# videosegmentation/video_segment

Measured on AMD Instinct MI355X. Metric: over-segmented frames/sec at 1080p, higher is better.
Workload: dtype f32

## Files before the change

video_segment_amd/csrc/merge_stage.hip:

```cpp
#include <sched.h>
#include <time.h>

#include <algorithm>
#include <atomic>
#include <chrono>
#include <thread>
#include <vector>

#include "merge_common.h"
#include "scan_device.h"

namespace vsg {

__global__ __launch_bounds__(256) void k_build_bucket_table(const ListDesc* __restrict__ lists,
                                                             int num_lists,
                                                             int32_t* __restrict__ bucket_base) {
  const int b = blockIdx.x * 256 + threadIdx.x;
  if (b > kNumBuckets) return;
  int acc = 0;
  int32_t* row = bucket_base + (size_t)b * (num_lists + 1);
  for (int l = 0; l < num_lists; ++l) {
    row[l] = acc;
    const int32_t* off = lists[l].offsets;
    if (off) acc += off[b + 1] - off[b];
  }
  row[num_lists] = acc;
}

void LaunchBuildBucketTable(const ListDesc* lists, int num_lists, int32_t* bucket_base,
                            hipStream_t s) {
  hipLaunchKernelGGL(k_build_bucket_table, dim3((kNumBuckets + 1 + 255) / 256), dim3(256), 0, s,
                     lists, num_lists, bucket_base);
  VSG_HIP(hipGetLastError());
}

__global__ __launch_bounds__(256) void k_init_identity(int32_t* a, size_t n) {
  const size_t i = (size_t)blockIdx.x * 256 + threadIdx.x;
  if (i < n) a[i] = (int32_t)i;
}

void LaunchInitIdentity(int32_t* a, size_t n, hipStream_t s) {
  hipLaunchKernelGGL(k_init_identity, dim3((unsigned)((n + 255) / 256)), dim3(256), 0, s, a, n);
  VSG_HIP(hipGetLastError());
}

__global__ void k_mail_post(unsigned long long* slot, unsigned seq, const int32_t* p0, const int32_t* p1,
                            const int32_t* p2, const int32_t* p3) {
  if (p0) MailPost(slot, seq, 0, *p0);
  if (p1) MailPost(slot, seq, 1, *p1);
  if (p2) MailPost(slot, seq, 2, *p2);
  if (p3) MailPost(slot, seq, 3, *p3);
}

void LaunchMailPost(const MailSlot& slot, const int32_t* p0, const int32_t* p1, const int32_t* p2,
                    const int32_t* p3, hipStream_t s) {
  hipLaunchKernelGGL(k_mail_post, dim3(1), dim3(1), 0, s, slot.dev, slot.seq, p0, p1, p2, p3);
  VSG_HIP(hipGetLastError());
}

static std::atomic<int> g_live_graphs{0};
void MailRegisterGraph(int delta) { g_live_graphs.fetch_add(delta, std::memory_order_relaxed); }

static int UsableCores() {
  cpu_set_t set;
  CPU_ZERO(&set);
  if (sched_getaffinity(0, sizeof(set), &set) == 0 && CPU_COUNT(&set) > 0) return (int)CPU_COUNT(&set);
  const unsigned h = std::thread::hardware_concurrency();
  return h ? (int)h : 1;
}

int MailYieldMode() {
  if (const char* e = getenv("VSG_MAIL_YIELD")) return std::max(0, std::min(2, atoi(e)));
  return 2 * g_live_graphs.load(std::memory_order_relaxed) > UsableCores() ? 1 : 0;
}

static thread_local MailWaitCounters t_mail_counters;
MailWaitCounters MailWaitSnapshot() { return t_mail_counters; }
void MailWaitResetLongest() { t_mail_counters.longest_ms = 0; }

namespace {
struct MailWaitTimer {
  std::chrono::steady_clock::time_point t0 = std::chrono::steady_clock::now();
  ~MailWaitTimer() {
    const double ms = std::chrono::duration<double, std::milli>(std::chrono::steady_clock::now() - t0).count();
    t_mail_counters.waits += 1;
    t_mail_counters.wait_ms += ms;
    if (ms > t_mail_counters.longest_ms) t_mail_counters.longest_ms = ms;
  }
};
}

void MailWait(const MailSlot& slot, int count, int* values, hipStream_t s) {
  using clk = std::chrono::steady_clock;
  MailWaitTimer wait_timer;
  clk::time_point t0;
  bool timed = false;
  const int mode = MailYieldMode();
  constexpr unsigned long long kBriefSpins = 512;
  long sleep_ns = 20000;
  for (int i = 0; i < count; ++i) {
    for (unsigned long long spins = 0;; ++spins) {
      const unsigned long long w = slot.host[i];
      if ((unsigned)(w >> 32) == slot.seq) {
        values[i] = (int)(unsigned)(w & 0xffffffffull);
        break;
      }
#if defined(__x86_64__)
      __builtin_ia32_pause();
#endif
      if (mode != 0 && spins >= kBriefSpins) {
        if (mode == 1) {
          std::this_thread::yield();
        } else {
          const timespec ts = {0, sleep_ns};
          nanosleep(&ts, nullptr);
          sleep_ns = std::min(sleep_ns * 2, 200000l);
        }
      }
      if ((mode == 0 && (spins & 0xffffull) == 0xffffull) || (mode != 0 && (spins & 0x3ffull) == 0x3ffull)) {
        const hipError_t e = hipStreamQuery(s);
        if (e != hipSuccess && e != hipErrorNotReady) VSG_HIP(e);
        if (!timed) {
          t0 = clk::now();
          timed = true;
        } else if (e == hipSuccess && clk::now() - t0 > std::chrono::seconds(2)) {
          const unsigned long long w2 = slot.host[i];
          if ((unsigned)(w2 >> 32) != slot.seq) throw Error(-4 , "mailbox: a value never arrived");
        }
        if (mode == 0) std::this_thread::yield();
      }
    }
  }
}

static void DrainStreams(MergeScratch& S) {
  VSG_HIP(hipStreamSynchronize(S.main_stream));
  if (S.aux_stream) VSG_HIP(hipStreamSynchronize(S.aux_stream));
  if (S.aux2_stream) VSG_HIP(hipStreamSynchronize(S.aux2_stream));
}

int32_t* TakeZeroed(MergeScratch& S, size_t n) {
  ZeroPool& z = *S.zeros;
  n = (n + 3) & ~(size_t)3;
  VSG_REQUIRE(z.cap > 2 * kZeroArenaInts, -4, "zero pool: too small");
  const size_t half = (z.cap - kZeroArenaInts) / 2;
  VSG_REQUIRE(n <= half, -4, "zero pool: request too large");
  if (z.used + n > half) {
    DrainStreams(S);
    z.second_half = !z.second_half;
    z.used = 0;
    VSG_HIP(hipMemsetAsync(z.base + kZeroArenaInts + (z.second_half ? half : 0), 0, half * sizeof(int32_t),
                           S.main_stream));
  }
  int32_t* p = z.base + kZeroArenaInts + (z.second_half ? half : 0) + z.used;
  z.used += n;
  return p;
}

int32_t* TakeStageScalars(MergeScratch& S, size_t n) {
  ZeroPool& z = *S.zeros;
  n = (n + 3) & ~(size_t)3;
  VSG_REQUIRE(n <= kZeroArenaInts, -4, "zero pool: stage scalars too large");
  if (z.arena_used + n > kZeroArenaInts) {
    DrainStreams(S);
    VSG_HIP(hipMemsetAsync(z.base, 0, kZeroArenaInts * sizeof(int32_t), S.main_stream));
    z.arena_used = 0;
  }
  int32_t* p = z.base + z.arena_used;
  z.arena_used += n;
  return p;
}

constexpr int kFilterPer = 2;
constexpr int kFilterEdges = 256 * kFilterPer;

__global__ __launch_bounds__(256) void k_filter(int bucket, int bucket_hi, int j0, int n_b,
                                                 const ListDesc* __restrict__ lists,
                                                 const int32_t* __restrict__ bucket_base,
                                                 const int32_t* __restrict__ bucket_prefix,
                                                 const uint32_t* __restrict__ list_slot_base,
                                                 uint8_t* __restrict__ kept_all, NodeArrays nodes,
                                                 MergeParams P, int inert_mode,
                                                 int32_t* __restrict__ cc,
                                                 int32_t* __restrict__ e_ra,
                                                 int32_t* __restrict__ e_rb,
                                                 uint32_t* __restrict__ e_gpos,
                                                 FilterMasks M,
                                                 int32_t* __restrict__ num_ti, FilterSegs segs, int hubs,
                                                 int32_t* __restrict__ num_hub, int32_t* __restrict__ hub_excl,
                                                 float split_s) {
  __shared__ int wave_cnt[kFilterPer][4], wave_kept[kFilterPer][4];
  __shared__ int s_start[kFilterEdges], s_pos0[kFilterEdges];
  __shared__ const uint32_t* s_slots[kFilterEdges];
  __shared__ const int32_t* s_prev[kFilterEdges];
  __shared__ int s_type[kFilterEdges], s_base_a[kFilterEdges], s_base_b[kFilterEdges];
  __shared__ uint32_t s_slot_base[kFilterEdges];
  const int jf = blockIdx.x * kFilterEdges;
  int m_segs = 0;
  if (segs.start) {
    int first = 0;
    if (segs.n > kFilterEdges) {
      const int stride = (segs.n + 255) / 256;
      const int t1 = threadIdx.x * stride;
      const int c1 = __syncthreads_count(t1 < segs.n && segs.start[t1] <= jf);
      const int base = (c1 - 1) * stride;
      const int t2 = base + threadIdx.x;
      const int c2 = __syncthreads_count(threadIdx.x < stride && t2 < segs.n && segs.start[t2] <= jf);
      first = base + c2 - 1;
    }
    m_segs = min(kFilterEdges, segs.n - first);
    for (int i = threadIdx.x; i < m_segs; i += 256) {
      s_start[i] = segs.start[first + i];
      const int l = segs.list[first + i];
      s_pos0[i] = segs.pos0[first + i];
      const ListDesc L = lists[l];
      s_slots[i] = L.slots;
      s_prev[i] = L.type != 0 ? L.prev_idx : reinterpret_cast<const int32_t*>(L.slots);
      s_type[i] = L.type;
      s_base_a[i] = L.base_a;
      s_base_b[i] = L.base_b;
      s_slot_base[i] = list_slot_base[l];
    }
    __syncthreads();
  }
  bool valid[kFilterPer];
  int a[kFilterPer], b[kFilterPer], l_type[kFilterPer];
  uint32_t gpos[kFilterPer];
  if (segs.start) {
    const uint32_t* slots_p[kFilterPer];
    const int32_t* prev_p[kFilterPer];
    int pos[kFilterPer], base_a[kFilterPer], base_b[kFilterPer];
#pragma unroll
    for (int e = 0; e < kFilterPer; ++e) {
      const int j = jf + e * 256 + threadIdx.x;
      valid[e] = j < n_b;
      const int jc = valid[e] ? j : n_b - 1;
      int lo = 0, hi = m_segs;
      while (hi - lo > 1) {
        const int mid = (lo + hi) >> 1;
        if (s_start[mid] <= jc) lo = mid; else hi = mid;
      }
      pos[e] = s_pos0[lo] + (jc - s_start[lo]);
      slots_p[e] = s_slots[lo];
      prev_p[e] = s_prev[lo];
      l_type[e] = s_type[lo];
      base_a[e] = s_base_a[lo];
      base_b[e] = s_base_b[lo];
      gpos[e] = s_slot_base[lo] + (uint32_t)pos[e];
    }
    uint32_t slot[kFilterPer];
#pragma unroll
    for (int e = 0; e < kFilterPer; ++e) slot[e] = slots_p[e][pos[e]];
    uint32_t pix[kFilterPer];
    int pv[kFilterPer];
#pragma unroll
    for (int e = 0; e < kFilterPer; ++e) {
      const uint32_t tm = (uint32_t)-(int)(l_type[e] != 0);
      pix[e] = ((slot[e] / 9u) & tm) | ((slot[e] >> 2) & ~tm);
      pv[e] = prev_p[e][pix[e]];
    }
#pragma unroll
    for (int e = 0; e < kFilterPer; ++e) {
      a[e] = base_a[e] + (int)pix[e];
      const int kt = (int)(slot[e] - pix[e] * 9u);
      const int dy = kt / 3 - 1, dx = kt - (kt / 3) * 3 - 1;
      const int bt = base_b[e] + pv[e] + dy * P.W + dx;
      const int ks = (int)(slot[e] & 3u);
      const int bs = a[e] + (ks != 0 ? P.W : 0) + (ks == 0 || ks == 3 ? 1 : 0) - (ks == 2 ? 1 : 0);
      const int tm = -(int)(l_type[e] != 0);
      b[e] = (bt & tm) | (bs & ~tm);
    }
  } else {
#pragma unroll
    for (int e = 0; e < kFilterPer; ++e) {
      const int j = jf + e * 256 + threadIdx.x;
      valid[e] = j < n_b;
      const int jc = valid[e] ? j : n_b - 1;
      int bk = bucket;
      int jb = j0 + jc;
      if (bucket_hi > bucket + 1) {
        const int jg = bucket_prefix[bucket] + jb;
        int lo = bucket, hi = bucket_hi;
        while (hi - lo > 1) {
          const int mid = (lo + hi) >> 1;
          if (bucket_prefix[mid] <= jg) lo = mid; else hi = mid;
        }
        bk = lo;
        jb = jg - bucket_prefix[bk];
      }
      const int32_t* base_row = bucket_base + (size_t)bk * (P.num_lists + 1);
      const int l = LocateList(base_row, P.num_lists, jb);
      const int pos = lists[l].offsets[bk] + (jb - base_row[l]);
      const ListDesc L = lists[l];
      l_type[e] = L.type;
      DecodeEdge(L, L.slots[pos], P.W, a[e], b[e]);
      gpos[e] = list_slot_base[l] + (uint32_t)pos;
    }
  }
  constexpr int kChains = 2 * kFilterPer;
  int x0[kChains], root[kChains];
#pragma unroll
  for (int e = 0; e < kFilterPer; ++e) {
    x0[2 * e] = a[e];
    x0[2 * e + 1] = b[e];
  }
#pragma unroll
  for (int c = 0; c < kChains; ++c) root[c] = x0[c];
  for (bool any = true; any;) {
    int p[kChains];
#pragma unroll
    for (int c = 0; c < kChains; ++c) p[c] = nodes.parent[root[c]];
    any = false;
#pragma unroll
    for (int c = 0; c < kChains; ++c) {
      if (p[c] != root[c]) {
        root[c] = p[c];
        any = true;
      }
    }
  }
  {
    int cur[kChains];
#pragma unroll
    for (int c = 0; c < kChains; ++c) cur[c] = x0[c];
    for (bool any = true; any;) {
      int nx[kChains];
#pragma unroll
      for (int c = 0; c < kChains; ++c) nx[c] = cur[c] != root[c] ? nodes.parent[cur[c]] : root[c];
      any = false;
#pragma unroll
      for (int c = 0; c < kChains; ++c) {
        if (cur[c] != root[c]) {
          if (nx[c] != root[c]) nodes.parent[cur[c]] = root[c];
          cur[c] = nx[c];
          any = any || (cur[c] != root[c]);
        }
      }
    }
  }
  int ti[kFilterPer], active[kFilterPer], settled[kFilterPer];
#pragma unroll
  for (int e = 0; e < kFilterPer; ++e) {
    ti[e] = active[e] = settled[e] = 0;
    const int ra = root[2 * e], rb = root[2 * e + 1];
    if (!valid[e] || ra == rb) continue;
    if (P.spatial_survivors && l_type[e] == 0 && !P.spatial_survivors[gpos[e]]) continue;
    bool inert = false;
    int f1 = 0, f2 = 0, s1 = 0, s2 = 0, c1 = -1, c2 = -1;
    if (inert_mode != 0) {
      f1 = nodes.flags[ra];
      f2 = nodes.flags[rb];
      if (f1 & kFlagFinalized) s1 = __float_as_int(nodes.desc_sz[ra].w);
      if (f2 & kFlagFinalized) s2 = __float_as_int(nodes.desc_sz[rb].w);
      const bool both_final_large = (f1 & kFlagFinalized) && (f2 & kFlagFinalized) &&
                                    (s1 >= P.min_region_size) && (s2 >= P.min_region_size);
      if (inert_mode == 1) {
        inert = both_final_large;
      } else {
        c1 = nodes.cons[ra];
        c2 = nodes.cons[rb];
        if (c1 >= 0 && c2 >= 0) {
          inert = (c1 != c2);
        } else {
          inert = both_final_large;
        }
        if (inert) {
          ti[e] = 1;
          if (!(f1 & kFlagTentative)) nodes.flags[ra] = (uint8_t)(f1 | kFlagTentative);
          if (!(f2 & kFlagTentative)) nodes.flags[rb] = (uint8_t)(f2 | kFlagTentative);
        }
      }
    }
    if (inert) {
      kept_all[gpos[e]] = 1;
      settled[e] = 1;
    } else {
      active[e] = 1;
      bool hub_edge = false;
      if (hubs) {
        constexpr int kNoHub = kFlagNoDesc | kFlagHubExcluded;
        const bool h1 = (f1 & kFlagFinalized) && !(f1 & kNoHub) && s1 >= P.min_region_size;
        const bool h2 = (f2 & kFlagFinalized) && !(f2 & kNoHub) && s2 >= P.min_region_size;
        if (h1 != h2) {
          const int h = h1 ? ra : rb, x = h1 ? rb : ra;
          const int fx = h1 ? f2 : f1, cx = h1 ? c2 : c1, fh = h1 ? f1 : f2;
          const int ch = h1 ? c1 : c2;
          if ((cx < 0 || cx == ch) && !(fx & kFlagNoDesc)) {
            hub_edge = true;
            root[2 * e] = x;
            root[2 * e + 1] = h;
            if (!nodes.hub8[h]) nodes.hub8[h] = 1;
            if (!(*num_hub & 1)) atomicOr(num_hub, 1);
            if (cx >= 0) {
              const float4 dx = nodes.desc_sz[x], dh = nodes.desc_sz[h];
              const float u = dh.x - dx.x, v = dh.y - dx.y, w = dh.z - dx.z;
              if ((u * u + v * v + w * w) * (1.0f / 3.0f) > split_s) {
                HubViolationAt(hub_excl, 0, jf + e * 256 + (int)threadIdx.x);
                if (!(*num_hub & 16)) atomicOr(num_hub, 16);
              }
            }
          } else {
            HubViolationAt(hub_excl, 0, jf + e * 256 + (int)threadIdx.x);
            if (!(fh & kFlagHubBroken)) HubExclude(hub_excl, nodes.flags, h);
          }
        } else if (h1 && h2) {
          HubViolationAt(hub_excl, 0, jf + e * 256 + (int)threadIdx.x);
          if (s1 <= s2 && !(f1 & kFlagHubBroken)) HubExclude(hub_excl, nodes.flags, ra);
          if (s2 <= s1 && !(f2 & kFlagHubBroken)) HubExclude(hub_excl, nodes.flags, rb);
        }
      }
      if (!hub_edge) CcUnion(cc, ra, rb);
    }
  }
  const int w = threadIdx.x >> 6, lane = threadIdx.x & 63;
  const int n_blocks = (n_b + 255) >> 8;
  unsigned long long ma[kFilterPer], ms[kFilterPer];
#pragma unroll
  for (int e = 0; e < kFilterPer; ++e) {
    ma[e] = __ballot(active[e] != 0);
    ms[e] = __ballot(settled[e] != 0);
    const unsigned long long mt = __ballot(ti[e] != 0);
    const int vb = blockIdx.x * kFilterPer + e;
    if (lane == 0 && vb < n_blocks) {
      const size_t gw = (size_t)vb * 4 + w;
      M.active[gw] = ma[e];
      M.settled[gw] = ms[e];
      M.tentative[gw] = mt;
      wave_cnt[e][w] = (int)__popcll(ma[e]);
      wave_kept[e][w] = (int)__popcll(ma[e] | ms[e]);
      if (mt != 0 && *num_ti == 0) *num_ti = 1;
    }
  }
  __syncthreads();
#pragma unroll
  for (int e = 0; e < kFilterPer; ++e) {
    const int vb = blockIdx.x * kFilterPer + e;
    if (active[e] | settled[e]) {
      int rank = (int)__popcll((ma[e] | ms[e]) & ((1ull << lane) - 1ull));
      for (int k = 0; k < w; ++k) rank += wave_kept[e][k];
      const int slot = vb * 256 + rank;
      e_ra[slot] = root[2 * e];
      e_rb[slot] = root[2 * e + 1];
      e_gpos[slot] = gpos[e];
    }
    if (threadIdx.x == 0 && vb < n_blocks) {
      M.block_cnt[vb] = wave_cnt[e][0] + wave_cnt[e][1] + wave_cnt[e][2] + wave_cnt[e][3];
    }
  }
}

__device__ __forceinline__ int FilterSlot(const FilterMasks& M, int j) {
  const int block = j >> 8, w = (j >> 6) & 3, lane = j & 63;
  const size_t gw0 = (size_t)block * 4;
  int rank = (int)__popcll((M.active[gw0 + w] | M.settled[gw0 + w]) & ((1ull << lane) - 1ull));
  for (int k = 0; k < w; ++k) rank += (int)__popcll(M.active[gw0 + k] | M.settled[gw0 + k]);
  return block * 256 + rank;
}

__global__ __launch_bounds__(256) void k_clear_tentative(int n_b, FilterMasks M,
                                                          const int32_t* __restrict__ e_ra,
                                                          const int32_t* __restrict__ e_rb,
                                                          NodeArrays nodes) {
  const int j = blockIdx.x * 256 + threadIdx.x;
  if (j >= n_b || !((M.tentative[j >> 6] >> (j & 63)) & 1ull)) return;
  const int slot = FilterSlot(M, j);
  int r[2] = {e_ra[slot], e_rb[slot]};
  for (int k = 0; k < 2; ++k) {
    int x = r[k];
    for (;;) {
      const int f = nodes.flags[x];
      if (f & kFlagTentative) nodes.flags[x] = (uint8_t)(f & ~kFlagTentative);
      const int p = nodes.parent[x];
      if (p == x) break;
      x = p;
    }
  }
}

__global__ __launch_bounds__(256) void k_backup_roots(int n, const int32_t* __restrict__ a_ra,
                                                       const int32_t* __restrict__ a_rb,
                                                       NodeArrays nodes, float4* __restrict__ bk_ds,
                                                       int32_t* __restrict__ bk_cons,
                                                       uint8_t* __restrict__ bk_flags,
                                                       unsigned long long* __restrict__ stats) {
  const int i = blockIdx.x * 256 + threadIdx.x;
  if (i < 8) stats[8 + i] = stats[i];
  if (i >= n) return;
  const int ra = a_ra[i], rb = a_rb[i];
  bk_ds[2 * i] = nodes.desc_sz[ra];
  bk_cons[2 * i] = nodes.cons[ra];
  bk_flags[2 * i] = nodes.flags[ra];
  bk_ds[2 * i + 1] = nodes.desc_sz[rb];
  bk_cons[2 * i + 1] = nodes.cons[rb];
  bk_flags[2 * i + 1] = nodes.flags[rb];
}

__global__ __launch_bounds__(256) void k_restore_roots(int n, const int32_t* __restrict__ a_ra,
                                                        const int32_t* __restrict__ a_rb,
                                                        NodeArrays nodes,
                                                        const float4* __restrict__ bk_ds,
                                                        const int32_t* __restrict__ bk_cons,
                                                        const uint8_t* __restrict__ bk_flags,
                                                        unsigned long long* __restrict__ stats) {
  const int i = blockIdx.x * 256 + threadIdx.x;
  if (i < 8) stats[i] = stats[8 + i];
  if (i >= n) return;
  const int ra = a_ra[i], rb = a_rb[i];
  nodes.parent[ra] = ra;
  nodes.desc_sz[ra] = bk_ds[2 * i];
  nodes.cons[ra] = bk_cons[2 * i];
  nodes.flags[ra] = bk_flags[2 * i];
  nodes.parent[rb] = rb;
  nodes.desc_sz[rb] = bk_ds[2 * i + 1];
  nodes.cons[rb] = bk_cons[2 * i + 1];
  nodes.flags[rb] = bk_flags[2 * i + 1];
}

__global__ __launch_bounds__(256) void k_clear_kept(int n_b, FilterMasks M,
                                                     const uint32_t* __restrict__ e_gpos,
                                                     uint8_t* __restrict__ kept_all) {
  const int j = blockIdx.x * 256 + threadIdx.x;
  if (j >= n_b) return;
  if (((M.active[j >> 6] | M.settled[j >> 6]) >> (j & 63)) & 1ull) kept_all[e_gpos[FilterSlot(M, j)]] = 0;
}

__global__ __launch_bounds__(256) void k_compact_active(int n_b, FilterMasks M,
                                                         const int32_t* __restrict__ block_off,
                                                         const int32_t* __restrict__ e_ra,
                                                         const int32_t* __restrict__ e_rb,
                                                         const uint32_t* __restrict__ e_gpos,
                                                         int32_t* __restrict__ a_ra,
                                                         int32_t* __restrict__ a_rb,
                                                         uint32_t* __restrict__ a_gpos,
                                                         int32_t* __restrict__ num_active,
                                                         const int32_t* __restrict__ num_ti,
                                                         unsigned long long* __restrict__ mail, unsigned mail_seq,
                                                         int a_cap, const int32_t* __restrict__ num_hub) {
  const int j = blockIdx.x * 256 + threadIdx.x;
  const int w = threadIdx.x >> 6, lane = threadIdx.x & 63;
  const size_t gw0 = (size_t)blockIdx.x * 4;
  const unsigned long long m = M.active[gw0 + w];
  int base = block_off[blockIdx.x];
  for (int k = 0; k < w; ++k) base += (int)__popcll(M.active[gw0 + k]);
  if ((m >> lane) & 1ull) {
    const int p = base + (int)__popcll(m & ((1ull << lane) - 1ull));
    if (p < a_cap) {
      const int slot = FilterSlot(M, j);
      a_ra[p] = e_ra[slot];
      a_rb[p] = e_rb[slot];
      a_gpos[p] = e_gpos[slot];
    }
  }
  if (blockIdx.x == gridDim.x - 1 && threadIdx.x == 255) {
    const int total = base + (int)__popcll(m);
    *num_active = total;
    MailPost(mail, mail_seq, 0, total);
    MailPost(mail, mail_seq, 1, *num_ti);
    MailPost(mail, mail_seq, 2, *num_hub);
  }
}

__global__ __launch_bounds__(256) void k_component_ids(int n, const int32_t* __restrict__ a_ra,
                                                        int32_t* __restrict__ cc,
                                                        uint32_t* __restrict__ a_comp,
                                                        uint32_t* __restrict__ a_idx) {
  const int i = blockIdx.x * 256 + threadIdx.x;
  if (i >= n) return;
  a_comp[i] = (uint32_t)CcFind(cc, a_ra[i]);
  a_idx[i] = (uint32_t)i;
}

__global__ __launch_bounds__(256) void k_reset_cc(int n, const int32_t* __restrict__ a_ra,
                                                   const int32_t* __restrict__ a_rb,
                                                   int32_t* __restrict__ cc,
                                                   const int32_t* __restrict__ violation,
                                                   unsigned long long* __restrict__ mail, unsigned mail_seq) {
  const int i = blockIdx.x * 256 + threadIdx.x;
  if (i == 0 && mail) MailPost(mail, mail_seq, 0, *violation);
  if (i >= n) return;
  const int ra = a_ra[i], rb = a_rb[i];
  cc[ra] = ra;
  cc[rb] = rb;
}

__global__ __launch_bounds__(256) void k_gather_sorted(int n, const uint32_t* __restrict__ s_idx,
                                                        const int32_t* __restrict__ a_ra,
                                                        const int32_t* __restrict__ a_rb,
                                                        const uint32_t* __restrict__ a_gpos,
                                                        int32_t* __restrict__ s_ra,
// ... 386 lines not shown
  for (int i = threadIdx.x; i < n; i += blockDim.x) at[i] = (int32_t)work_gpos[at[i]];
}
void ResetHubExclusions(MergeScratch& S, NodeArrays nodes, hipStream_t s) {
  if (!S.hub_excl) return;
  hipLaunchKernelGGL(k_hub_unexclude, dim3(16), dim3(256), 0, s, S.hub_excl, nodes);
  hipLaunchKernelGGL(k_hub_excl_reset, dim3(1), dim3(1), 0, s, S.hub_excl);
  VSG_HIP(hipGetLastError());
}

__global__ void k_plain_edge(int bucket, int jb, const ListDesc* __restrict__ lists,
                             const int32_t* __restrict__ bucket_base, const uint32_t* __restrict__ list_slot_base,
                             uint8_t* __restrict__ kept_all, NodeArrays nodes, MergeParams P, StageThr T,
                             unsigned long long* __restrict__ stats) {
  const int32_t* base_row = bucket_base + (size_t)bucket * (P.num_lists + 1);
  const int l = LocateList(base_row, P.num_lists, jb);
  const int pos = lists[l].offsets[bucket] + (jb - base_row[l]);
  const ListDesc L = lists[l];
  int a, b;
  DecodeEdge(L, L.slots[pos], P.W, a, b);
  const uint32_t gpos = list_slot_base[l] + (uint32_t)pos;
  if (P.spatial_survivors && L.type == 0 && !P.spatial_survivors[gpos]) return;
  int r1 = a, r2 = b;
  for (int p; (p = nodes.parent[r1]) != r1;) r1 = p;
  for (int p; (p = nodes.parent[r2]) != r2;) r2 = p;
  if (r1 == r2) return;
  RState s1 = LoadState(nodes, r1), s2 = LoadState(nodes, r2);
  int stat;
  const int out = DecideEdge(s1, s2, T, stat);
  if (stat >= 1 && stat <= 3) atomicAdd(&stats[stat - 1], 1ull);
  if (out == kOutKeep) {
    kept_all[gpos] = 1;
    StoreState(nodes, r1, s1);
    StoreState(nodes, r2, s2);
  } else if (out == kOutMerge1) {
    StoreState(nodes, r1, s1);
    nodes.parent[r2] = r1;
  } else {
    StoreState(nodes, r2, s2);
    nodes.parent[r1] = r2;
  }
}

static long long SequencePosition(const MergeScratch& S, const MergeParams& P, int b_lo, int b_hi, uint32_t gpos) {
  const int L = P.num_lists;
  int lo = 0, hi = L;
  while (hi - lo > 1) {
    const int mid = (lo + hi) >> 1;
    if (S.list_slot_base_host[mid] <= gpos) lo = mid; else hi = mid;
  }
  const int l = lo;
  const long long p = (long long)gpos - (long long)S.list_slot_base_host[l];
  const int32_t* off = S.list_off_host + (size_t)l * (kNumBuckets + 2);
  int b0 = b_lo, b1 = b_hi;
  while (b1 - b0 > 1) {
    const int mid = (b0 + b1) >> 1;
    if (off[mid] <= p) b0 = mid; else b1 = mid;
  }
  const int32_t* row = S.bucket_base_host + (size_t)b0 * (L + 1);
  return (long long)S.bucket_prefix_host[b0] + row[l] + (p - (long long)off[b0]);
}
static int BucketOfPosition(const MergeScratch& S, int b_lo, int b_hi, long long g) {
  int b0 = b_lo, b1 = b_hi;
  while (b1 - b0 > 1) {
    const int mid = (b0 + b1) >> 1;
    if ((long long)S.bucket_prefix_host[mid] <= g) b0 = mid; else b1 = mid;
  }
  return b0;
}

static inline unsigned Blocks(int n) { return (unsigned)((n + 255) / 256); }

__global__ void k_max_segment(int max_segs, const int32_t* __restrict__ num_segs,
                              const int32_t* __restrict__ seg_cnt, int below, int32_t* __restrict__ out);

void RunBucketStage(int bucket, int j0, int n_b, const ListDesc* lists, const int32_t* bucket_base,
                    const uint32_t* list_slot_base, uint8_t* kept_all, NodeArrays nodes,
                    const MergeParams& P, int inert_mode, MergeScratch& S, hipStream_t s,
                    StageInfo* info) {
  if (info) {
    info->replayed = 0;
    info->components = 0;
  }
  if (n_b <= 0) return;
  const int bucket_hi = S.group_hi > bucket ? S.group_hi : bucket + 1;
  int32_t* d_num_ti = TakeStageScalars(S, 8);
  int32_t* d_violation = d_num_ti + 1;
  int32_t* d_num_hub = d_num_ti + 2;
  int32_t* d_hub_count = d_num_ti + 3;
  int32_t* d_hub_runs = d_num_ti + 4;
  const bool spine_possible = S.spine_min > 0 && !S.spine_off && bucket < *S.spine_limit_bucket &&
                              !(bucket < 2 && S.spine_low_skip[bucket]);
  const bool try_hubs = S.hubs && !S.hubs_off && inert_mode != 0 && !spine_possible && S.wide_min <= 0;
  if (S.hub_excl && S.hub_list_dirty) {
    if (S.hub_attempt == 0) {
      VSG_HIP(hipMemsetAsync(S.hub_excl, 0, 4 * sizeof(int32_t), s));
      S.hub_list_dirty = 0;
    } else {
      VSG_HIP(hipMemsetAsync(S.hub_excl + 1, 0, 3 * sizeof(int32_t), s));
    }
  }
  if (S.hub_excl && S.hub_check) {
    int head[4] = {0, 0, 0, 0};
    VSG_HIP(hipMemcpyAsync(head, S.hub_excl, sizeof(head), hipMemcpyDeviceToHost, s));
    VSG_HIP(hipStreamSynchronize(s));
    for (int k = 1; k < 4; ++k) {
      if (head[k] != 0) {
        Throw(-4 , "hub check: stage b=" + std::to_string(bucket) + " j0=" + std::to_string(j0) +
                                             " n=" + std::to_string(n_b) + " starts with " + std::to_string(head[k]) +
                                             " stale entries of kind " + std::to_string(k - 1) + " on the hub list");
      }
    }
  }
  if (S.hub_attempt == 0 && S.hub_split_depth == 0) S.hub_splits_left = S.hub_max_splits;
  int32_t* d_num_leaders = S.num_active + 5;
  FilterSegs segs = {nullptr, nullptr, nullptr, 0};
  if (S.bucket_base_host && S.list_off_host && S.seg_dev) {
    const int L = P.num_lists;
    std::vector<int32_t>& h = *S.seg_host;
    h.clear();
    const int64_t g0 = (int64_t)S.bucket_prefix_host[bucket] + j0, g1 = g0 + n_b;
    std::vector<int32_t> st, li, po;
    for (int b = bucket; b < bucket_hi; ++b) {
      const int32_t* row = S.bucket_base_host + (size_t)b * (L + 1);
      const int64_t bstart = S.bucket_prefix_host[b];
      if (bstart + row[L] <= g0) continue;
      if (bstart >= g1) break;
      for (int l = 0; l < L; ++l) {
        const int cnt = row[l + 1] - row[l];
        if (cnt == 0) continue;
        const int64_t s0 = bstart + row[l], s1 = s0 + cnt;
        if (s1 <= g0 || s0 >= g1) continue;
        const int64_t first = std::max(s0, g0);
        st.push_back((int32_t)(first - g0));
        li.push_back(l);
        po.push_back(S.list_off_host[(size_t)l * (kNumBuckets + 2) + b] + (int32_t)(first - s0));
      }
    }
    const int nseg = (int)st.size();
    if (nseg > 0 && nseg <= 65536 && (size_t)3 * nseg <= S.seg_cap) {
      h.reserve((size_t)3 * nseg);
      h.insert(h.end(), st.begin(), st.end());
      h.insert(h.end(), li.begin(), li.end());
      h.insert(h.end(), po.begin(), po.end());
      VSG_HIP(hipMemcpyAsync(S.seg_dev, h.data(), h.size() * sizeof(int32_t), hipMemcpyHostToDevice, s));
      segs.start = S.seg_dev;
      segs.list = S.seg_dev + nseg;
      segs.pos0 = S.seg_dev + 2 * (size_t)nseg;
      segs.n = nseg;
    }
  }
  const float split_s = ((float)bucket * P.inv_scale < P.force_merge_weight) ? P.s_lt_02 : P.s_le_015;
  const int ef0 = NextEvent(S);
  if (ef0 >= 0) VSG_HIP(hipEventRecord((*S.ev_pool)[ef0], s));
  hipLaunchKernelGGL(k_filter, dim3((unsigned)((n_b + kFilterEdges - 1) / kFilterEdges)), dim3(256), 0, s, bucket, bucket_hi, j0, n_b, lists,
                     bucket_base, S.bucket_prefix, list_slot_base, kept_all, nodes, P, inert_mode, S.cc, S.e_ra, S.e_rb, S.e_gpos,
                     S.masks, d_num_ti, segs, try_hubs ? 1 : 0, d_num_hub, S.hub_excl, split_s);
  const int ef1 = NextEvent(S);
  if (ef1 >= 0) {
    VSG_HIP(hipEventRecord((*S.ev_pool)[ef1], s));
    S.ev_filter->emplace_back(ef0, ef1);
  }
  if (try_hubs) hipLaunchKernelGGL(k_hub_check, dim3(16), dim3(256), 0, s, S.hub_excl, nodes, d_num_hub);
  ExclusiveSum(S.scan, S.masks.block_cnt, S.block_off, (int)Blocks(n_b), s);
  int h[3] = {0, 0, 0};
  for (int attempt = 0;; ++attempt) {
    const MailSlot m_active = NextMail(*S.mail);
    hipLaunchKernelGGL(k_compact_active, dim3(Blocks(n_b)), dim3(256), 0, s, n_b, S.masks, S.block_off,
                       S.e_ra, S.e_rb, S.e_gpos, S.a_ra, S.a_rb, S.a_gpos, S.num_active, d_num_ti, m_active.dev,
                       m_active.seq, S.active_cap, d_num_hub);
    VSG_HIP(hipGetLastError());
    MailWait(m_active, 3, h, s);
    if (h[0] <= S.active_cap) break;
    VSG_REQUIRE(attempt == 0 && S.grow_active && S.grow_active(h[0]) && h[0] <= S.active_cap, -4,
                "stage scratch: cannot hold the active edges");
  }
  const int n_active = h[0];
  const int n_ti = h[1];
  const bool hubs_used = try_hubs && (h[2] & 1) != 0;
  if (h[2] & (8 | 16)) S.hub_list_dirty = 1;
  auto clear_hub_marks = [&]() {
    if (try_hubs && (h[2] & 9) != 0 && n_active > 0) {
      hipLaunchKernelGGL(k_hub_clear, dim3(Blocks(n_active)), dim3(256), 0, s, n_active, S.a_ra, S.a_rb, nodes);
    }
  };
  auto clear_marks = [&]() {
    if (n_ti > 0) {
      hipLaunchKernelGGL(k_clear_tentative, dim3(Blocks(n_b)), dim3(256), 0, s, n_b, S.masks, S.e_ra,
                         S.e_rb, nodes);
    }
  };
  if (n_active == 0) {
    clear_marks();
    return;
  }
  auto can_cut = [&](int work, long long violations) {
    return work >= S.hub_cut_min_work && (long long)n_b > S.hub_cut_ratio * (violations + 1) && S.hub_splits_left > 0 &&
           S.bucket_base_host && S.bucket_prefix_host && S.list_off_host && S.list_slot_base_host;
  };
  auto retry_without_broken_hubs = [&](int violated, int work, bool list_complete, const uint32_t* work_gpos) -> bool {
    for (int q = 0; q < 6; ++q) S.hub_reasons[q] += (violated >> (2 + q)) & 1;
    ++S.hub_retries;
    if (info) ++info->hub_retries;
    std::vector<int> cuts;
    const long long g_stage = (long long)S.bucket_prefix_host[bucket] + j0;
    int head[4] = {0, 0, 0, 0};
    if (can_cut(work, 0)) {
      VSG_HIP(hipMemcpyAsync(head, S.hub_excl, sizeof(head), hipMemcpyDeviceToHost, s));
      VSG_HIP(hipStreamSynchronize(s));
    }
    if (can_cut(work, (long long)head[1] + (work_gpos ? head[2] + head[3] : 0))) {
      int at[3 * kHubCutCap];
      int raw1[kHubCutCap];
      if (S.hub_check && work_gpos) {
        VSG_HIP(hipMemcpyAsync(raw1, S.hub_excl + 4 + kHubExclCap + kHubCutCap, sizeof(raw1), hipMemcpyDeviceToHost, s));
        VSG_HIP(hipStreamSynchronize(s));
        for (int i = 0; i < std::min(head[2], kHubCutCap); ++i) {
          if (raw1[i] < 0 || raw1[i] >= work) {
            Throw(-4 , "hub check: stage b=" + std::to_string(bucket) + " j0=" + std::to_string(j0) +
                                                 " n=" + std::to_string(n_b) + ": cut entry " + std::to_string(i) +
                                                 " of kind 1 is work edge " + std::to_string(raw1[i]) + " of " +
                                                 std::to_string(work));
          }
        }
      }
      if (work_gpos) hipLaunchKernelGGL(k_hub_cut_gpos, dim3(1), dim3(64), 0, s, S.hub_excl, work_gpos);
      VSG_HIP(hipMemcpyAsync(at, S.hub_excl + 4 + kHubExclCap, sizeof(at), hipMemcpyDeviceToHost, s));
      VSG_HIP(hipStreamSynchronize(s));
      auto check_at = [&](int kind, int i, long long v, long long lo, long long hi) {
        if (S.hub_check && (v < lo || v >= hi)) {
          Throw(-4 , "hub check: stage b=" + std::to_string(bucket) + " j0=" + std::to_string(j0) +
                                               " n=" + std::to_string(n_b) + ": cut entry " + std::to_string(i) +
                                               " of kind " + std::to_string(kind) + " is " + std::to_string(v) +
                                               ", outside [" + std::to_string(lo) + ", " + std::to_string(hi) + ")");
        }
      };
      auto in_stage = [&](int kind, int i, uint32_t gpos) {
        if (!S.hub_check) return;
        const long long g = SequencePosition(S, P, bucket, bucket_hi, gpos) - g_stage;
        check_at(kind, i, g, 0, n_b);
        const long long gg = g_stage + g;
        const int b = BucketOfPosition(S, bucket, bucket_hi, gg);
        const int32_t* row = S.bucket_base_host + (size_t)b * (P.num_lists + 1);
        const int jb = (int)(gg - S.bucket_prefix_host[b]);
        int l = 0;
        while (l + 1 < P.num_lists && row[l + 1] <= jb) ++l;
        if ((uint32_t)(S.list_slot_base_host[l] + S.list_off_host[(size_t)l * (kNumBuckets + 2) + b] + (jb - row[l])) != gpos) {
          Throw(-4 , "hub check: stage b=" + std::to_string(bucket) + " j0=" + std::to_string(j0) +
                                               " n=" + std::to_string(n_b) + ": cut entry " + std::to_string(i) +
                                               " of kind " + std::to_string(kind) + " is kept position " +
                                               std::to_string(gpos) + ", not an edge of the stage");
        }
      };
      for (int i = 0; i < std::min(head[1], kHubCutCap); ++i) {
        check_at(0, i, at[i], 0, n_b);
        cuts.push_back(at[i]);
      }
      if (work_gpos) {
        for (int i = 0; i < std::min(head[2], kHubCutCap); ++i) {
          in_stage(1, i, (uint32_t)at[kHubCutCap + i]);
          cuts.push_back((int)(SequencePosition(S, P, bucket, bucket_hi, (uint32_t)at[kHubCutCap + i]) - g_stage));
        }
        for (int i = 0; i < std::min(head[3], kHubCutCap); ++i) {
          in_stage(2, i, (uint32_t)at[2 * kHubCutCap + i]);
          cuts.push_back((int)(SequencePosition(S, P, bucket, bucket_hi, (uint32_t)at[2 * kHubCutCap + i]) - g_stage));
        }
      }
      std::sort(cuts.begin(), cuts.end());
      cuts.erase(std::unique(cuts.begin(), cuts.end()), cuts.end());
      while (!cuts.empty() && cuts.back() >= n_b) cuts.pop_back();
      while (!cuts.empty() && cuts.front() < 0) cuts.erase(cuts.begin());
      if (!work_gpos && cuts.size() > 1) cuts.resize(1);
      if ((int)cuts.size() > S.hub_splits_left) cuts.resize((size_t)S.hub_splits_left);
    }
    if (getenv("VSG_DEBUG_STAGES")) {
      int cnt = 0;
      VSG_HIP(hipMemcpyAsync(&cnt, S.hub_excl, sizeof(int), hipMemcpyDeviceToHost, s));
      VSG_HIP(hipStreamSynchronize(s));
      std::fprintf(stderr, "[vsg]   hub rule violated (mask %x) in b=%d j0=%d n=%d work %d, attempt %d, %d regions on the "
                   "list, %zu cuts (first at %d, %d left)\n", violated, bucket, j0, n_b, work, S.hub_attempt, cnt,
                   cuts.size(), cuts.empty() ? -1 : cuts[0], S.hub_splits_left);
    }
    if (!cuts.empty()) {
      S.hub_splits_left -= (int)cuts.size();
      S.hub_splits += (long long)cuts.size();
      if (bucket_hi > bucket + 1) S.hub_cuts_in_groups += (long long)cuts.size();
      if (violated == 2 && bucket < 2) S.spine_side_cuts += (long long)cuts.size();
      int replayed = 0;
      auto part = [&](int off, int n, bool plain) {
        if (n <= 0) return;
        StageInfo sub;
        if (info) sub.want_components = info->want_components;
        ++S.hub_split_depth;
        if (plain) ++S.hubs_off;
        const int b_at = BucketOfPosition(S, bucket, bucket_hi, g_stage + off);
        if (b_at > bucket) ++S.hub_parts_in_later_bucket;
        RunBucketStage(b_at, (int)(g_stage + off - S.bucket_prefix_host[b_at]), n, lists, bucket_base, list_slot_base,
                       kept_all, nodes, P, inert_mode, S, s, info ? &sub : nullptr);
        if (plain) --S.hubs_off;
        --S.hub_split_depth;
        replayed += sub.replayed;
        if (info) {
          info->hub_stages += sub.hub_stages;
          info->hub_absorbed += sub.hub_absorbed;
          info->hub_retries += sub.hub_retries;
          info->components += sub.components;
          info->max_wave_segment = std::max(info->max_wave_segment, sub.max_wave_segment);
        }
      };
      StageThr plain;
// ... 342 lines not shown
```

Measured before the change: 196.6.

## Template filter kernel on edges per thread and overlap root-finding loads

Makes k_filter a template on edges per thread and raises the default from 2 to 4. The segment table is capped at 256 entries, with a global binary-search fallback for edges past it. The first parent loads are issued early to overlap with decode, and path compression reuses the first two hops already read. Per-root flag, size and constraint loads are batched ahead of the decision logic, and duplicate unions between adjacent lanes are skipped. Env-gated per-thread override and a stats probe are added; larger PER raises register pressure and makes tentative-flag updates need cross-edge checks.

```diff
diff --git a/video_segment_amd/csrc/merge_stage.hip b/video_segment_amd/csrc/merge_stage.hip
--- a/video_segment_amd/csrc/merge_stage.hip
+++ b/video_segment_amd/csrc/merge_stage.hip
@@ -2,6 +2,9 @@
 #include <time.h>
 
 #include <algorithm>
+#include <climits>
+#include <cstdio>
+#include <cstdlib>
 #include <atomic>
 #include <chrono>
 #include <thread>
@@ -171,9 +174,11 @@
   return p;
 }
 
-constexpr int kFilterPer = 2;
-constexpr int kFilterEdges = 256 * kFilterPer;
-
+constexpr int kFilterPer = 4;
+constexpr int kFilterSegTab = 256;
+enum FilterStat { kFsEdges, kFsInternal, kFsActive, kFsSettled, kFsHops, kFsHopMax, kFsSegMiss, kFsCount };
+
+template <int PER>
 __global__ __launch_bounds__(256) void k_filter(int bucket, int bucket_hi, int j0, int n_b,
                                                  const ListDesc* __restrict__ lists,
                                                  const int32_t* __restrict__ bucket_base,
@@ -188,18 +193,18 @@
                                                  FilterMasks M,
                                                  int32_t* __restrict__ num_ti, FilterSegs segs, int hubs,
                                                  int32_t* __restrict__ num_hub, int32_t* __restrict__ hub_excl,
-                                                 float split_s) {
-  __shared__ int wave_cnt[kFilterPer][4], wave_kept[kFilterPer][4];
-  __shared__ int s_start[kFilterEdges], s_pos0[kFilterEdges];
-  __shared__ const uint32_t* s_slots[kFilterEdges];
-  __shared__ const int32_t* s_prev[kFilterEdges];
-  __shared__ int s_type[kFilterEdges], s_base_a[kFilterEdges], s_base_b[kFilterEdges];
-  __shared__ uint32_t s_slot_base[kFilterEdges];
-  const int jf = blockIdx.x * kFilterEdges;
-  int m_segs = 0;
+                                                 float split_s, int32_t* __restrict__ fstats) {
+  constexpr int kEdges = 256 * PER;
+  __shared__ int wave_cnt[PER][4], wave_kept[PER][4];
+  __shared__ int s_start[kFilterSegTab], s_pos0[kFilterSegTab];
+  __shared__ const uint32_t* s_slots[kFilterSegTab];
+  __shared__ const int32_t* s_prev[kFilterSegTab];
+  __shared__ int s_type[kFilterSegTab], s_base_a[kFilterSegTab], s_base_b[kFilterSegTab];
+  __shared__ uint32_t s_slot_base[kFilterSegTab];
+  const int jf = blockIdx.x * kEdges;
+  int m_segs = 0, first = 0, next_start = INT_MAX;
   if (segs.start) {
-    int first = 0;
-    if (segs.n > kFilterEdges) {
+    if (segs.n > kFilterSegTab) {
       const int stride = (segs.n + 255) / 256;
       const int t1 = threadIdx.x * stride;
       const int c1 = __syncthreads_count(t1 < segs.n && segs.start[t1] <= jf);
@@ -208,7 +213,8 @@
       const int c2 = __syncthreads_count(threadIdx.x < stride && t2 < segs.n && segs.start[t2] <= jf);
       first = base + c2 - 1;
     }
-    m_segs = min(kFilterEdges, segs.n - first);
+    m_segs = min(kFilterSegTab, segs.n - first);
+    if (first + m_segs < segs.n) next_start = segs.start[first + m_segs];
     for (int i = threadIdx.x; i < m_segs; i += 256) {
       s_start[i] = segs.start[first + i];
       const int l = segs.list[first + i];
@@ -223,45 +229,65 @@
     }
     __syncthreads();
   }
-  bool valid[kFilterPer];
-  int a[kFilterPer], b[kFilterPer], l_type[kFilterPer];
-  uint32_t gpos[kFilterPer];
+  bool valid[PER];
+  int a[PER], b[PER], l_type[PER], pa[PER], pb[PER];
+  uint32_t gpos[PER];
+  int seg_miss = 0;
   if (segs.start) {
-    const uint32_t* slots_p[kFilterPer];
-    const int32_t* prev_p[kFilterPer];
-    int pos[kFilterPer], base_a[kFilterPer], base_b[kFilterPer];
-#pragma unroll
-    for (int e = 0; e < kFilterPer; ++e) {
+    const uint32_t* slots_p[PER];
+    const int32_t* prev_p[PER];
+    int pos[PER], base_a[PER], base_b[PER];
+#pragma unroll
+    for (int e = 0; e < PER; ++e) {
       const int j = jf + e * 256 + threadIdx.x;
       valid[e] = j < n_b;
       const int jc = valid[e] ? j : n_b - 1;
-      int lo = 0, hi = m_segs;
-      while (hi - lo > 1) {
-        const int mid = (lo + hi) >> 1;
-        if (s_start[mid] <= jc) lo = mid; else hi = mid;
-      }
-      pos[e] = s_pos0[lo] + (jc - s_start[lo]);
-      slots_p[e] = s_slots[lo];
-      prev_p[e] = s_prev[lo];
-      l_type[e] = s_type[lo];
-      base_a[e] = s_base_a[lo];
-      base_b[e] = s_base_b[lo];
-      gpos[e] = s_slot_base[lo] + (uint32_t)pos[e];
-    }
-    uint32_t slot[kFilterPer];
-#pragma unroll
-    for (int e = 0; e < kFilterPer; ++e) slot[e] = slots_p[e][pos[e]];
-    uint32_t pix[kFilterPer];
-    int pv[kFilterPer];
-#pragma unroll
-    for (int e = 0; e < kFilterPer; ++e) {
+      if (jc < next_start) {
+        int lo = 0, hi = m_segs;
+        while (hi - lo > 1) {
+          const int mid = (lo + hi) >> 1;
+          if (s_start[mid] <= jc) lo = mid; else hi = mid;
+        }
+        pos[e] = s_pos0[lo] + (jc - s_start[lo]);
+        slots_p[e] = s_slots[lo];
+        prev_p[e] = s_prev[lo];
+        l_type[e] = s_type[lo];
+        base_a[e] = s_base_a[lo];
+        base_b[e] = s_base_b[lo];
+        gpos[e] = s_slot_base[lo] + (uint32_t)pos[e];
+      } else {
+        int lo = first + m_segs, hi = segs.n;
+        while (hi - lo > 1) {
+          const int mid = (lo + hi) >> 1;
+          if (segs.start[mid] <= jc) lo = mid; else hi = mid;
+        }
+        const int l = segs.list[lo];
+        const ListDesc L = lists[l];
+        pos[e] = segs.pos0[lo] + (jc - segs.start[lo]);
+        slots_p[e] = L.slots;
+        prev_p[e] = L.type != 0 ? L.prev_idx : reinterpret_cast<const int32_t*>(L.slots);
+        l_type[e] = L.type;
+        base_a[e] = L.base_a;
+        base_b[e] = L.base_b;
+        gpos[e] = list_slot_base[l] + (uint32_t)pos[e];
+        seg_miss += valid[e] ? 1 : 0;
+      }
+    }
+    uint32_t slot[PER];
+#pragma unroll
+    for (int e = 0; e < PER; ++e) slot[e] = slots_p[e][pos[e]];
+    uint32_t pix[PER];
+    int pv[PER];
+#pragma unroll
+    for (int e = 0; e < PER; ++e) {
       const uint32_t tm = (uint32_t)-(int)(l_type[e] != 0);
       pix[e] = ((slot[e] / 9u) & tm) | ((slot[e] >> 2) & ~tm);
+      a[e] = base_a[e] + (int)pix[e];
       pv[e] = prev_p[e][pix[e]];
-    }
-#pragma unroll
-    for (int e = 0; e < kFilterPer; ++e) {
-      a[e] = base_a[e] + (int)pix[e];
+      pa[e] = nodes.parent[a[e]];
+    }
+#pragma unroll
+    for (int e = 0; e < PER; ++e) {
       const int kt = (int)(slot[e] - pix[e] * 9u);
       const int dy = kt / 3 - 1, dx = kt - (kt / 3) * 3 - 1;
       const int bt = base_b[e] + pv[e] + dy * P.W + dx;
@@ -269,10 +295,11 @@
       const int bs = a[e] + (ks != 0 ? P.W : 0) + (ks == 0 || ks == 3 ? 1 : 0) - (ks == 2 ? 1 : 0);
       const int tm = -(int)(l_type[e] != 0);
       b[e] = (bt & tm) | (bs & ~tm);
+      pb[e] = nodes.parent[b[e]];
     }
   } else {
 #pragma unroll
-    for (int e = 0; e < kFilterPer; ++e) {
+    for (int e = 0; e < PER; ++e) {
       const int j = jf + e * 256 + threadIdx.x;
       valid[e] = j < n_b;
       const int jc = valid[e] ? j : n_b - 1;
@@ -296,25 +323,40 @@
       DecodeEdge(L, L.slots[pos], P.W, a[e], b[e]);
       gpos[e] = list_slot_base[l] + (uint32_t)pos;
     }
-  }
-  constexpr int kChains = 2 * kFilterPer;
-  int x0[kChains], root[kChains];
-#pragma unroll
-  for (int e = 0; e < kFilterPer; ++e) {
+#pragma unroll
+    for (int e = 0; e < PER; ++e) {
+      pa[e] = nodes.parent[a[e]];
+      pb[e] = nodes.parent[b[e]];
+    }
+  }
+  constexpr int kChains = 2 * PER;
+  int x0[kChains], root[kChains], n1[kChains], n2[kChains], hops[kChains];
+#pragma unroll
+  for (int e = 0; e < PER; ++e) {
     x0[2 * e] = a[e];
     x0[2 * e + 1] = b[e];
-  }
-#pragma unroll
-  for (int c = 0; c < kChains; ++c) root[c] = x0[c];
-  for (bool any = true; any;) {
+    n1[2 * e] = pa[e];
+    n1[2 * e + 1] = pb[e];
+  }
+  bool any = false;
+#pragma unroll
+  for (int c = 0; c < kChains; ++c) {
+    root[c] = n1[c];
+    n2[c] = n1[c];
+    hops[c] = n1[c] != x0[c] ? 1 : 0;
+    any = any || hops[c] != 0;
+  }
+  for (int it = 0; any; ++it) {
     int p[kChains];
 #pragma unroll
     for (int c = 0; c < kChains; ++c) p[c] = nodes.parent[root[c]];
     any = false;
 #pragma unroll
     for (int c = 0; c < kChains; ++c) {
+      if (it == 0) n2[c] = p[c];
       if (p[c] != root[c]) {
         root[c] = p[c];
+        ++hops[c];
         any = true;
       }
     }
@@ -322,52 +364,84 @@
   {
     int cur[kChains];
 #pragma unroll
-    for (int c = 0; c < kChains; ++c) cur[c] = x0[c];
-    for (bool any = true; any;) {
+    for (int c = 0; c < kChains; ++c) {
+      if (n1[c] != root[c]) nodes.parent[x0[c]] = root[c];
+      if (n1[c] != root[c] && n2[c] != root[c]) nodes.parent[n1[c]] = root[c];
+      cur[c] = n2[c];
+    }
+    for (bool more = true; more;) {
       int nx[kChains];
 #pragma unroll
       for (int c = 0; c < kChains; ++c) nx[c] = cur[c] != root[c] ? nodes.parent[cur[c]] : root[c];
-      any = false;
+      more = false;
 #pragma unroll
       for (int c = 0; c < kChains; ++c) {
         if (cur[c] != root[c]) {
           if (nx[c] != root[c]) nodes.parent[cur[c]] = root[c];
           cur[c] = nx[c];
-          any = any || (cur[c] != root[c]);
-        }
-      }
-    }
-  }
-  int ti[kFilterPer], active[kFilterPer], settled[kFilterPer];
-#pragma unroll
-  for (int e = 0; e < kFilterPer; ++e) {
+          more = more || (cur[c] != root[c]);
+        }
+      }
+    }
+  }
+  bool need[PER];
+  int f1[PER], f2[PER], s1[PER], s2[PER], c1[PER], c2[PER], surv[PER];
+#pragma unroll
+  for (int e = 0; e < PER; ++e) {
+    const int ra = root[2 * e], rb = root[2 * e + 1];
+    need[e] = valid[e] && ra != rb;
+    f1[e] = f2[e] = s1[e] = s2[e] = 0;
+    c1[e] = c2[e] = -1;
+    surv[e] = 1;
+    if (need[e]) {
+      if (P.spatial_survivors && l_type[e] == 0) surv[e] = P.spatial_survivors[gpos[e]];
+      if (inert_mode != 0) {
+        f1[e] = nodes.flags[ra];
+        f2[e] = nodes.flags[rb];
+        s1[e] = __float_as_int(nodes.desc_sz[ra].w);
+        s2[e] = __float_as_int(nodes.desc_sz[rb].w);
+        if (inert_mode == 2) {
+          c1[e] = nodes.cons[ra];
+          c2[e] = nodes.cons[rb];
+        }
+      }
+    }
+  }
+  int ti[PER], active[PER], settled[PER];
+  bool join[PER];
+#pragma unroll
+  for (int e = 0; e < PER; ++e) {
     ti[e] = active[e] = settled[e] = 0;
+    join[e] = false;
     const int ra = root[2 * e], rb = root[2 * e + 1];
-    if (!valid[e] || ra == rb) continue;
-    if (P.spatial_survivors && l_type[e] == 0 && !P.spatial_survivors[gpos[e]]) continue;
+    if (!need[e]) continue;
+    if (!surv[e]) continue;
     bool inert = false;
-    int f1 = 0, f2 = 0, s1 = 0, s2 = 0, c1 = -1, c2 = -1;
+    const int f1e = f1[e], f2e = f2[e], c1e = c1[e], c2e = c2[e];
+    const int s1e = (f1e & kFlagFinalized) ? s1[e] : 0, s2e = (f2e & kFlagFinalized) ? s2[e] : 0;
     if (inert_mode != 0) {
-      f1 = nodes.flags[ra];
-      f2 = nodes.flags[rb];
-      if (f1 & kFlagFinalized) s1 = __float_as_int(nodes.desc_sz[ra].w);
-      if (f2 & kFlagFinalized) s2 = __float_as_int(nodes.desc_sz[rb].w);
-      const bool both_final_large = (f1 & kFlagFinalized) && (f2 & kFlagFinalized) &&
-                                    (s1 >= P.min_region_size) && (s2 >= P.min_region_size);
+      const bool both_final_large = (f1e & kFlagFinalized) && (f2e & kFlagFinalized) &&
+                                    (s1e >= P.min_region_size) && (s2e >= P.min_region_size);
       if (inert_mode == 1) {
         inert = both_final_large;
       } else {
-        c1 = nodes.cons[ra];
-        c2 = nodes.cons[rb];
-        if (c1 >= 0 && c2 >= 0) {
-          inert = (c1 != c2);
+        if (c1e >= 0 && c2e >= 0) {
+          inert = (c1e != c2e);
         } else {
           inert = both_final_large;
         }
         if (inert) {
           ti[e] = 1;
-          if (!(f1 & kFlagTentative)) nodes.flags[ra] = (uint8_t)(f1 | kFlagTentative);
-          if (!(f2 & kFlagTentative)) nodes.flags[rb] = (uint8_t)(f2 | kFlagTentative);
+          bool seen1 = false, seen2 = false;
+#pragma unroll
+          for (int k = 0; k < e; ++k) {
+            seen1 = seen1 || ra == root[2 * k] || ra == root[2 * k + 1];
+            seen2 = seen2 || rb == root[2 * k] || rb == root[2 * k + 1];
+          }
+          const int g1 = seen1 ? (int)nodes.flags[ra] : f1e;
+          const int g2 = seen2 ? (int)nodes.flags[rb] : f2e;
+          if (!(g1 & kFlagTentative)) nodes.flags[ra] = (uint8_t)(g1 | kFlagTentative);
+          if (!(g2 & kFlagTentative)) nodes.flags[rb] = (uint8_t)(g2 | kFlagTentative);
         }
       }
     }
@@ -379,12 +453,12 @@
       bool hub_edge = false;
       if (hubs) {
         constexpr int kNoHub = kFlagNoDesc | kFlagHubExcluded;
-        const bool h1 = (f1 & kFlagFinalized) && !(f1 & kNoHub) && s1 >= P.min_region_size;
-        const bool h2 = (f2 & kFlagFinalized) && !(f2 & kNoHub) && s2 >= P.min_region_size;
+        const bool h1 = (f1e & kFlagFinalized) && !(f1e & kNoHub) && s1e >= P.min_region_size;
+        const bool h2 = (f2e & kFlagFinalized) && !(f2e & kNoHub) && s2e >= P.min_region_size;
         if (h1 != h2) {
           const int h = h1 ? ra : rb, x = h1 ? rb : ra;
-          const int fx = h1 ? f2 : f1, cx = h1 ? c2 : c1, fh = h1 ? f1 : f2;
-          const int ch = h1 ? c1 : c2;
+          const int fx = h1 ? f2e : f1e, cx = h1 ? c2e : c1e, fh = h1 ? f1e : f2e;
+          const int ch = h1 ? c1e : c2e;
           if ((cx < 0 || cx == ch) && !(fx & kFlagNoDesc)) {
             hub_edge = true;
             root[2 * e] = x;
@@ -405,22 +479,30 @@
           }
         } else if (h1 && h2) {
           HubViolationAt(hub_excl, 0, jf + e * 256 + (int)threadIdx.x);
-          if (s1 <= s2 && !(f1 & kFlagHubBroken)) HubExclude(hub_excl, nodes.flags, ra);
-          if (s2 <= s1 && !(f2 & kFlagHubBroken)) HubExclude(hub_excl, nodes.flags, rb);
-        }
-      }
-      if (!hub_edge) CcUnion(cc, ra, rb);
-    }
+          if (s1e <= s2e && !(f1e & kFlagHubBroken)) HubExclude(hub_excl, nodes.flags, ra);
+          if (s2e <= s1e && !(f2e & kFlagHubBroken)) HubExclude(hub_excl, nodes.flags, rb);
+        }
+      }
+      join[e] = !hub_edge;
+    }
+  }
+#pragma unroll
+  for (int e = 0; e < PER; ++e) {
+    const int ra = root[2 * e], rb = root[2 * e + 1];
+    const int qa = __shfl_up(ra, 1), qb = __shfl_up(rb, 1);
+    const bool qj = __shfl_up((int)join[e], 1) != 0;
+    const bool dup = (threadIdx.x & 63) != 0 && qj && ((qa == ra && qb == rb) || (qa == rb && qb == ra));
+    if (join[e] && !dup) CcUnion(cc, ra, rb);
   }
   const int w = threadIdx.x >> 6, lane = threadIdx.x & 63;
   const int n_blocks = (n_b + 255) >> 8;
-  unsigned long long ma[kFilterPer], ms[kFilterPer];
-#pragma unroll
-  for (int e = 0; e < kFilterPer; ++e) {
+  unsigned long long ma[PER], ms[PER];
+#pragma unroll
+  for (int e = 0; e < PER; ++e) {
     ma[e] = __ballot(active[e] != 0);
     ms[e] = __ballot(settled[e] != 0);
     const unsigned long long mt = __ballot(ti[e] != 0);
-    const int vb = blockIdx.x * kFilterPer + e;
+    const int vb = blockIdx.x * PER + e;
     if (lane == 0 && vb < n_blocks) {
       const size_t gw = (size_t)vb * 4 + w;
       M.active[gw] = ma[e];
@@ -431,10 +513,28 @@
       if (mt != 0 && *num_ti == 0) *num_ti = 1;
     }
   }
+  if (fstats) {
+    int v[kFsCount] = {};
+#pragma unroll
+    for (int e = 0; e < PER; ++e) {
+      if (!valid[e]) continue;
+      v[kFsEdges] += 1;
+      v[kFsInternal] += root[2 * e] == root[2 * e + 1] ? 1 : 0;
+      v[kFsActive] += active[e];
+      v[kFsSettled] += settled[e];
+      v[kFsHops] += hops[2 * e] + hops[2 * e + 1];
+      v[kFsHopMax] = max(v[kFsHopMax], max(hops[2 * e], hops[2 * e + 1]));
+    }
+    v[kFsSegMiss] = seg_miss;
+#pragma unroll
+    for (int k = 0; k < kFsCount; ++k) {
+      if (k == kFsHopMax) atomicMax(&fstats[k], v[k]); else if (v[k]) atomicAdd(&fstats[k], v[k]);
+    }
+  }
   __syncthreads();
 #pragma unroll
-  for (int e = 0; e < kFilterPer; ++e) {
-    const int vb = blockIdx.x * kFilterPer + e;
+  for (int e = 0; e < PER; ++e) {
+    const int vb = blockIdx.x * PER + e;
     if (active[e] | settled[e]) {
       int rank = (int)__popcll((ma[e] | ms[e]) & ((1ull << lane) - 1ull));
       for (int k = 0; k < w; ++k) rank += wave_kept[e][k];
@@ -1127,9 +1227,35 @@
   const float split_s = ((float)bucket * P.inv_scale < P.force_merge_weight) ? P.s_lt_02 : P.s_le_015;
   const int ef0 = NextEvent(S);
   if (ef0 >= 0) VSG_HIP(hipEventRecord((*S.ev_pool)[ef0], s));
-  hipLaunchKernelGGL(k_filter, dim3((unsigned)((n_b + kFilterEdges - 1) / kFilterEdges)), dim3(256), 0, s, bucket, bucket_hi, j0, n_b, lists,
-                     bucket_base, S.bucket_prefix, list_slot_base, kept_all, nodes, P, inert_mode, S.cc, S.e_ra, S.e_rb, S.e_gpos,
-                     S.masks, d_num_ti, segs, try_hubs ? 1 : 0, d_num_hub, S.hub_excl, split_s);
+  const char* per_env = getenv("VSG_FILTER_PER");
+  const int per = per_env ? atoi(per_env) : kFilterPer;
+  VSG_REQUIRE(per == 2 || per == 4 || per == 8, -4, "VSG_FILTER_PER: 2, 4 or 8");
+  int32_t* fstats = getenv("VSG_FILTER_STATS") ? TakeZeroed(S, kFsCount) : nullptr;
+  const dim3 fgrid((unsigned)((n_b + 256 * per - 1) / (256 * per)));
+#define VSG_LAUNCH_FILTER(PER)                                                                                    \
+  hipLaunchKernelGGL(k_filter<PER>, fgrid, dim3(256), 0, s, bucket, bucket_hi, j0, n_b, lists, bucket_base,       \
+                     S.bucket_prefix, list_slot_base, kept_all, nodes, P, inert_mode, S.cc, S.e_ra, S.e_rb,       \
+                     S.e_gpos, S.masks, d_num_ti, segs, try_hubs ? 1 : 0, d_num_hub, S.hub_excl, split_s, fstats)
+  if (per == 2) {
+    VSG_LAUNCH_FILTER(2);
+  } else if (per == 4) {
+    VSG_LAUNCH_FILTER(4);
+  } else {
+    VSG_LAUNCH_FILTER(8);
+  }
+#undef VSG_LAUNCH_FILTER
+  if (fstats) {
+    int32_t v[kFsCount];
+    VSG_HIP(hipMemcpyAsync(v, fstats, sizeof(v), hipMemcpyDeviceToHost, s));
+    VSG_HIP(hipStreamSynchronize(s));
+    std::fprintf(stderr,
+                 "[vsg] filter: buckets %d-%d j0=%d n_b=%d per=%d decode=%s segs=%d inert=%d hubs=%d | internal=%d "
+                 "active=%d settled=%d hops mean=%.3f max=%d seg_misses=%d\n",
+                 bucket, bucket_hi - 1, j0, n_b, per, segs.start ? "segments" : "search", segs.n, inert_mode,
+                 try_hubs ? 1 : 0, v[kFsInternal], v[kFsActive], v[kFsSettled],
+                 v[kFsEdges] ? (double)v[kFsHops] / (2.0 * v[kFsEdges]) : 0.0, v[kFsHopMax], v[kFsSegMiss]);
+    VSG_REQUIRE(v[kFsEdges] == n_b, -4, "filter stats: edge count");
+  }
   const int ef1 = NextEvent(S);
   if (ef1 >= 0) {
     VSG_HIP(hipEventRecord((*S.ev_pool)[ef1], s));
```

Measured after the change: 199.7, median of 6. +1.6%, better.
